# ccchengff/SketchML

Measured on AMD Instinct MI355X. Metric: device-resident grad encode GB/s (fp32 in) + decode L2 err, 1/2/4/8 GPU, higher is better.
Workload: dtype f32; 1 GPU; north star: 2^28-float dense gradient bucket per GPU, 256 requested bins, encode; n_per_gpu=268435456, bins=256, rotating_buffers=2, parallelism=dp1

## Files before the change

include/skml.h:

```cpp
#ifndef SKML_H
#define SKML_H

#include <stddef.h>
#include <stdint.h>

#ifdef __cplusplus
extern "C" {
#endif

#define SKML_OK 0
#define SKML_E_ARG 1
#define SKML_E_NAN 2
#define SKML_E_ORDER 3
#define SKML_E_HIP 4
#define SKML_E_RCCL 5
#define SKML_E_OOM 6
#define SKML_E_STATE 7

#define SKML_DENSE_MAGIC 0x444D4B53u
#define SKML_MAX_BINS 65536

typedef struct skml_ctx skml_ctx;

typedef struct skml_params {
// ... 41 lines not shown
#define SKML_K_DECODE 4
#define SKML_K_DECODE_SUM 5
#define SKML_K_SPARSE 6
#define SKML_K_COUNT 7
#define SKML_TIMING_ALL (-1)
int skml_ctx_set_timing(skml_ctx* ctx, int mask);
int skml_ctx_kernel_stats(skml_ctx* ctx, int kid, int64_t* launches, double* total_ms);
int skml_ctx_reset_stats(skml_ctx* ctx);
int skml_debug_leaf_stage(skml_ctx* ctx, const float* x_dev, int64_t n, int stage, int iters,
                          double* avg_ms);
int skml_debug_sparse_scratch_fail(int on);

int skml_debug_sparse_merge_path(void);

#define SKML_FORM_LEAF_SPLIT 0
#define SKML_FORM_DECODE_SUM 1
#define SKML_FORM_PART_BALLOT 2
#define SKML_FORM_RS_ROUNDS 3
#define SKML_FORM_DEC_ROWS_SERIAL 4
#define SKML_FORM_AGG_TILES 5
#define SKML_FORM_AGG_ONE_LANE 6
#define SKML_FORM_RUN_BOUNDS 7
#define SKML_FORM_DEC_LOOKBACK 8
#define SKML_FORM_COUNT 9
int skml_debug_form(int id, int value);
#define SKML_BUILD_AB 1
int skml_build_flags(void);


size_t skml_dense_payload_bytes(int64_t n, int32_t bin_num);

int skml_dense_encode_f32(skml_ctx* ctx, const float* x_dev, int64_t n, const skml_params* params,
                          void* payload_dev, size_t payload_cap);

int skml_dense_encode_f64(skml_ctx* ctx, const double* x_dev, int64_t n, const skml_params* params,
                          void* payload_dev, size_t payload_cap);

int skml_dense_encode_bf16(skml_ctx* ctx, const uint16_t* x_dev, int64_t n, const skml_params* params,
                           void* payload_dev, size_t payload_cap);
int skml_dense_encode_f16(skml_ctx* ctx, const uint16_t* x_dev, int64_t n, const skml_params* params,
                          void* payload_dev, size_t payload_cap);

int skml_dense_encode_uniform_f32(skml_ctx* ctx, const float* x_dev, int64_t n,
                                  const skml_params* params, void* payload_dev, size_t payload_cap);
int skml_dense_encode_uniform_f64(skml_ctx* ctx, const double* x_dev, int64_t n,
                                  const skml_params* params, void* payload_dev, size_t payload_cap);

// ... 186 lines not shown
```

sketchml_amd/_lib.py:

```python
from __future__ import annotations

import contextlib
import ctypes as C
import os

import torch

_HERE = os.path.dirname(os.path.abspath(__file__))
LIB_PATH = os.environ.get("SKML_LIB", os.path.join(_HERE, "lib", "libskml.so"))

SKML_OK = 0
SKML_E_ARG = 1
SKML_E_NAN = 2
SKML_E_ORDER = 3
SKML_E_HIP = 4
SKML_E_RCCL = 5
SKML_E_OOM = 6
SKML_E_STATE = 7
UNIQUE_ID_BYTES = 128
SKML_MAX_BINS = 65536
SKML_FIXED_MAGIC = 0x584D4B53
SKML_QUANTILE = 0
SKML_UNIFORM = 1

# ... 142 lines not shown
    "skml_comm_init_rank": (C.c_int, [vp, u8p, i32, i32, C.POINTER(vp)]),
    "skml_comm_destroy": (C.c_int, [vp]),
    "skml_allgather": (C.c_int, [vp, vp, vp, C.c_size_t, vp]),
}

EXPORTED = tuple(_SIGS)


def _load():
    if not os.path.exists(LIB_PATH):
        raise ImportError(f"sketchml_amd: HIP library not built ({LIB_PATH}); run "
                          f"`python -c 'import __graft_entry__ as g; g.build()'`")
    lib = C.CDLL(LIB_PATH)
    for name, (res, args) in _SIGS.items():
        fn = getattr(lib, name)
        fn.restype = res
        fn.argtypes = args
    return lib


lib = _load()

FORMS = {"leaf_split": 0, "decode_sum": 1, "part_ballot": 2, "rs_rounds": 3, "dec_rows_serial": 4,
         "agg_tiles": 5, "agg_one_lane": 6, "run_bounds": 7, "dec_lookback": 8}


AB_BUILD = bool(lib.skml_build_flags() & 1)


class FormNotBuilt(RuntimeError):
    """A kernel form only the A/B build carries (skml_debug_form returned -2)."""


@contextlib.contextmanager
def forced_forms(**values):
    prev = {}
    try:
        for k, v in values.items():
            r = lib.skml_debug_form(FORMS[k], int(v))
            if r == -2:
                raise FormNotBuilt(f"form {k}={v} is built only with -DSKML_AB (SKML_LIB=sketchml_amd/lib_ab/libskml.so)")
            if r < 0:
                raise ValueError(f"unknown form {k}")
            prev[k] = r
        yield
    finally:
        for k, v in prev.items():
# ... 6 lines not shown
```

sketchml_amd/csrc/skml_api.cpp:

```cpp
#include <hip/hip_runtime.h>
#include <rccl/rccl.h>

#include <atomic>
#include <cmath>
#include <condition_variable>
#include <cstdarg>
#include <cstdio>
#include <cstdlib>
#include <cstring>
#include <functional>
#include <mutex>
#include <string>
#include <thread>
#include <vector>

#include "skml_internal.h"
#include "skml_sparse.h"

using namespace skml;

namespace {

thread_local std::string g_err;

// ... 10 lines not shown
#define HIP_TRY(expr)                                                                       \
    do {                                                                                    \
        hipError_t e_ = (expr);                                                             \
        if (e_ != hipSuccess)                                                               \
            return fail(SKML_E_HIP, "%s failed: %s (%s:%d)", #expr, hipGetErrorString(e_), \
                        __FILE__, __LINE__);                                                \
    } while (0)

}

struct skml_ctx {
    int device = 0;
    hipStream_t stream = nullptr;
    bool own_stream = false;
    uint64_t* jump_tab = nullptr;
    void* ws = nullptr;
    size_t ws_cap = 0;
    void* ws64 = nullptr;
    size_t ws64_cap = 0;
    int64_t* ranks = nullptr;
    size_t ranks_cap = 0;
    int64_t ranks_n = -1;
    int ranks_bins = -1;
    skml_ctx* side = nullptr;
    hipEvent_t ev_join = nullptr, ev_leaf = nullptr;
    hipEvent_t ev_fork2 = nullptr, ev_join2 = nullptr;
    hipEvent_t after_leaf = nullptr;
    hipEvent_t ev_switch = nullptr;
    void* sk = nullptr;
    size_t sk_cap = 0;
    FxPartial* fx_part = nullptr;
    void* stage = nullptr;
    size_t stage_cap = 0;
    void* scratch[kScratchSlots] = {};
    size_t scratch_cap[kScratchSlots] = {};
    void* pinned = nullptr;
    size_t pinned_cap = 0;
    int64_t* hword = nullptr;
    void* hx = nullptr;
    size_t hx_cap = 0;
    void* hp = nullptr;
    size_t hp_cap = 0;
    void* hk = nullptr;
    size_t hk_cap = 0;
    void* hpin[2] = {nullptr, nullptr};
    size_t hpin_cap = 0;
// ... 25 lines not shown
    }
    ~KernelTimer() {
        if (!on) return;
        (void)hipEventRecord(c->ev[kid][c->ev_used[kid] + 1], c->stream);
        c->ev_used[kid] += 2;
    }
};
KernelTimer* make_timer(skml_ctx* c, int kid) { return new KernelTimer(c, kid); }
void end_timer(KernelTimer* t) { delete t; }

static std::atomic<int> g_form[SKML_FORM_COUNT];
int form(int id) { return id >= 0 && id < SKML_FORM_COUNT ? g_form[id].load(std::memory_order_relaxed) : 0; }
}

static bool ab_only_form(int id, int v) {
    switch (id) {
        case SKML_FORM_LEAF_SPLIT: return v == 1 || v >= 3;
        case SKML_FORM_DECODE_SUM: return v == 2;
        case SKML_FORM_RS_ROUNDS: return v == 2;
        case SKML_FORM_DEC_ROWS_SERIAL: return v == 2;
        case SKML_FORM_AGG_TILES: return v >= 2;
        case SKML_FORM_RUN_BOUNDS: return v != 0;
        case SKML_FORM_DEC_LOOKBACK: return v != 0;
        default: return false;
    }
}

extern "C" int skml_debug_form(int id, int value) {
    if (id < 0 || id >= SKML_FORM_COUNT) return -1;
#ifndef SKML_AB
    if (ab_only_form(id, value)) return -2;
#else
    (void)ab_only_form;
#endif
    return g_form[id].exchange(value);
}

extern "C" int skml_build_flags(void) {
#ifdef SKML_AB
    return SKML_BUILD_AB;
#else
    return 0;
#endif
}

namespace {

struct Workspace {
    unsigned* done;
    LeafPartial* part;
    float* nodes6;
    float* roots;
    float* upA;
    float* upB;
    double* raw;
    QuantLut* lut;
    UniPartial* uni;
    int* qflags;
    uint8_t* ubits;
    LeafPartial* part_red;
};

size_t ws_layout(int64_t chunks, Workspace* w, char* base) {
    const int64_t nwg = (chunks + kLeafChunks - 1) / kLeafChunks;
    const int64_t full = chunks / kLeafChunks;
    const int64_t up = (full >> kMergeGroupLog) + 2 * kMaxLevels + 8;
    size_t off = 0;
    auto take = [&](size_t bytes) {
        size_t o = off;
        off = align_up(off + bytes, 256);
        return base ? (void*)(base + o) : nullptr;
    };
    Workspace t;
    t.done = (unsigned*)take(256);
    t.part = (LeafPartial*)take(sizeof(LeafPartial) * (size_t)(nwg + 1));
    t.nodes6 = (float*)take(sizeof(float) * kK * (size_t)(full + 1));
    t.roots = (float*)take(sizeof(float) * kK * kMaxLevels);
    t.upA = (float*)take(sizeof(float) * kK * (size_t)up);
    t.upB = (float*)take(sizeof(float) * kK * (size_t)up);
    t.raw = (double*)take(sizeof(double) * SKML_MAX_BINS);
    t.lut = (QuantLut*)take(sizeof(QuantLut));
    t.uni = (UniPartial*)take(sizeof(UniPartial) * kUniMaxParts);
    t.qflags = (int*)take(sizeof(int) * 4);
    t.ubits = (uint8_t*)take((size_t)upper_node_count(full * kLeafChunks) + 64);
    t.part_red = (LeafPartial*)take(sizeof(LeafPartial) * (size_t)(full + 8));
    if (w) *w = t;
    return off;
}

int ensure_ws(skml_ctx* ctx, int64_t chunks, Workspace* w) {
    const size_t need = ws_layout(chunks, nullptr, nullptr);
    if (need > ctx->ws_cap) {
        if (ctx->ws) HIP_TRY(hipFree(ctx->ws));
        ctx->ws = nullptr;
        size_t cap = need + need / 4;
        HIP_TRY(hipMalloc(&ctx->ws, cap));
        HIP_TRY(hipMemsetAsync(ctx->ws, 0, 256, ctx->stream));
        ctx->ws_cap = cap;
    }
    ws_layout(chunks, w, (char*)ctx->ws);
    return SKML_OK;
}

struct Workspace64 {
    LeafPartial64* part;
    double* nodes6;
    double* roots;
    double* upA;
    double* upB;
    double* raw;
    uint8_t* ubits;
};

size_t ws64_layout(int64_t chunks, Workspace64* w, char* base) {
    const int64_t tiles = (chunks + kLeafChunks - 1) / kLeafChunks;
    const int64_t up = (tiles >> 3) + 8;
    size_t off = 0;
    auto take = [&](size_t bytes) {
        size_t o = off;
        off = align_up(off + bytes, 256);
// ... 55 lines not shown
        uint64_t a = 1, c = 0;
        for (int b = 0; b < 256; b++) {
            tab[(lvl * 256 + b) * 2] = a;
            tab[(lvl * 256 + b) * 2 + 1] = c;
            c = (base_a * c + base_c) & kLcgMask;
            a = (base_a * a) & kLcgMask;
        }
        uint64_t na = 1, nc = 0;
        for (int i = 0; i < 256; i++) {
            nc = (base_a * nc + base_c) & kLcgMask;
            na = (base_a * na) & kLcgMask;
        }
        base_a = na;
        base_c = nc;
    }
}

struct Tree {
    int level;
    int m;
    int cur_level;
    int64_t src;
    int64_t chunk_base;
};

bool valid_payload_ptr(const void* p) { return p && (((uintptr_t)p) % 256 == 0); }

void destroy_host_path(skml_ctx* c);

}

extern "C" {

void skml_params_default(skml_params* p) {
    p->bin_num = 256;
    p->group_num = 8;
    p->row_num = 2;
    p->dedup = 1;
    p->col_ratio = 0.3;
    p->seed = 0;
    p->hash_seed = 0;
    p->quant_type = SKML_QUANTILE;
    p->parallelism = 1;
}

const char* skml_last_error(void) { return g_err.c_str(); }
// ... 25 lines not shown
    void* pin = e == hipSuccess ? skml::ctx_pinned(c, tab_bytes) : nullptr;
    if (e == hipSuccess && !pin) e = hipErrorOutOfMemory;
    if (e == hipSuccess) {
        std::memcpy(pin, tab.data(), tab_bytes);
        e = hipMemcpyAsync(c->jump_tab, pin, tab_bytes, hipMemcpyHostToDevice, c->stream);
    }
    if (e == hipSuccess) e = hipStreamSynchronize(c->stream);
    if (e != hipSuccess) {
        skml_ctx_destroy(c);
        return fail(SKML_E_HIP, "jump table: %s", hipGetErrorString(e));
    }
    *out = c;
    return SKML_OK;
}

int skml_ctx_destroy(skml_ctx* c) {
    if (!c) return SKML_OK;
    (void)hipSetDevice(c->device);
    if (c->stream) (void)hipStreamSynchronize(c->stream);
    if (c->jump_tab) (void)hipFree(c->jump_tab);
    if (c->ws) (void)hipFree(c->ws);
    if (c->ws64) (void)hipFree(c->ws64);
    if (c->ranks) (void)hipFree(c->ranks);
    if (c->stage) (void)hipFree(c->stage);
    if (c->side) skml_ctx_destroy(c->side);
    if (c->ev_join) (void)hipEventDestroy(c->ev_join);
    if (c->ev_leaf) (void)hipEventDestroy(c->ev_leaf);
    if (c->ev_fork2) (void)hipEventDestroy(c->ev_fork2);
    if (c->ev_join2) (void)hipEventDestroy(c->ev_join2);
    if (c->ev_switch) (void)hipEventDestroy(c->ev_switch);
    if (c->sk) (void)hipFree(c->sk);
    if (c->fx_part) (void)hipFree(c->fx_part);
    for (int k = 0; k < SKML_K_COUNT; k++)
        for (hipEvent_t e : c->ev[k]) (void)hipEventDestroy(e);
    for (int i = 0; i < kScratchSlots; i++)
        if (c->scratch[i]) (void)hipFree(c->scratch[i]);
    if (c->pinned) (void)hipHostFree(c->pinned);
    if (c->hword) (void)hipHostFree(c->hword);
    destroy_host_path(c);
    if (c->own_stream) (void)hipStreamDestroy(c->stream);
    delete c;
    return SKML_OK;
}

int skml_ctx_sync(skml_ctx* c) {
    if (!c) return fail(SKML_E_ARG, "ctx is NULL");
// ... 79 lines not shown
size_t skml_dense_payload_bytes(int64_t n, int32_t bin_num) {
    if (n < 0 || bin_num < 2 || bin_num > SKML_MAX_BINS) return 0;
    const size_t rounded = align_up((size_t)n, 1024);
    return dense_codes_offset(bin_num) + align_up(rounded * (size_t)code_bits_for(bin_num) / 8, 256);
}

static int check_dense_args(skml_ctx* c, const void* x, int64_t n, int bins, const void* payload,
                            size_t cap) {
    if (!c) return fail(SKML_E_ARG, "ctx is NULL");
    if (n < 0 || n > 0x7FFFFFFFLL) return fail(SKML_E_ARG, "n=%lld outside Java int range", (long long)n);
    if (bins < 2 || bins > SKML_MAX_BINS)
        return fail(SKML_E_ARG, "Invalid partition number: %d", bins);
    if (n > 0 && (!x || ((uintptr_t)x) % 16 != 0))
        return fail(SKML_E_ARG, "input must be a 16-byte aligned device pointer");
    if (!valid_payload_ptr(payload)) return fail(SKML_E_ARG, "payload must be 256-byte aligned");
    if (cap < skml_dense_payload_bytes(n, bins))
        return fail(SKML_E_ARG, "payload capacity %zu < %zu", cap, skml_dense_payload_bytes(n, bins));
    return SKML_OK;
}

}

namespace {
std::vector<MergePass> plan_merge_passes(int64_t chunks) {
    std::vector<Tree> trees;
    for (int l = kMaxLevels - 1; l > kLeafTopLevel; l--) {
        if (!((chunks >> l) & 1)) continue;
        Tree t;
        t.level = l;
        t.m = l - kLeafTopLevel;
        t.cur_level = kLeafTopLevel;
        t.chunk_base = (chunks >> (l + 1)) << (l + 1);
        t.src = t.chunk_base >> kLeafTopLevel;
        trees.push_back(t);
    }
    std::vector<MergePass> passes;
    while (true) {
        MergePass pass;
        std::memset(&pass, 0, sizeof(pass));
        int64_t dst_off = 0;
        int wg = 0;
        for (auto& t : trees) {
            if (t.m == 0) continue;
            const int g = t.m < kMergeGroupLog ? t.m : kMergeGroupLog;
            MergeJob& j = pass.job[pass.njobs];
            j.src_node = t.src;
            j.dst_node = dst_off;
            j.chunk_base = t.chunk_base;
            j.level_in = t.cur_level;
            j.group_log = g;
            j.groups = 1 << (t.m - g);
            j.root_level = (t.m - g == 0) ? t.level : -1;
            pass.wg_prefix[pass.njobs] = wg;
            wg += j.groups;
            pass.njobs++;
            t.src = dst_off;
            dst_off += j.groups;
            t.m -= g;
            t.cur_level += g;
        }
        if (pass.njobs == 0) break;
        pass.wg_prefix[pass.njobs] = wg;
        passes.push_back(pass);
    }
    return passes;
}
constexpr int kFuseMaxWg = 4;
bool fuse_next_pass(const std::vector<MergePass>& passes, size_t i) {
    return i + 2 == passes.size() && passes[i + 1].wg_prefix[passes[i + 1].njobs] <= kFuseMaxWg;
}
}

namespace {
int run_sketch_f32(skml_ctx* c, const void* x, int64_t n, uint64_t s0, const Workspace& w, const skml_params* p,
                   void* payload, bool summary, bool* fused_out, int xtype = kXF32) {
    const int64_t chunks = n / kChunk;
    const int64_t nwg = (chunks + kLeafChunks - 1) / kLeafChunks;
    bool fused = false;
    if (chunks > 0) {
        {
            KernelTimer kt(c, SKML_K_LEAF);
            HIP_TRY(launch_leaf(c->stream, x, chunks, s0, c->jump_tab, w.part, w.nodes6, w.roots, w.ubits, xtype));
        }
        if (c->after_leaf) {
            HIP_TRY(hipEventRecord(c->after_leaf, c->stream));
            c->after_leaf = nullptr;
        }
        std::vector<MergePass> passes = plan_merge_passes(chunks);
        if (summary && !passes.empty()) passes.back().fuse_summary = 1;
        const int64_t nred = passes.empty() ? 0 : passes[0].wg_prefix[passes[0].njobs];
        const int64_t part_from = passes.empty() ? 0 : (chunks >> 7) << 1;
        const float* src = w.nodes6;
        float* dst = w.upA;
        for (size_t i = 0; i < passes.size(); i++) {
            const bool fuse_next = fuse_next_pass(passes, i);
            float* next_dst = (dst == w.upA) ? w.upB : w.upA;
            KernelTimer kt(c, SKML_K_MERGE);
            HIP_TRY(launch_merge_pass(c->stream, passes[i], fuse_next ? &passes[i + 1] : nullptr, src, dst, next_dst,
                                      w.roots, s0, c->jump_tab, w.done, x, n, w.part, nwg, c->ranks, p->bin_num,
                                      p->dedup ? 1 : 0, payload, w.raw, w.lut, w.ubits,
                                      summary ? w.part_red : nullptr, summary ? nred : 0, summary ? part_from : 0,
                                      xtype));
            src = dst;
            dst = next_dst;
            if (fuse_next) break;
        }
        fused = summary && !passes.empty();
    }
    *fused_out = fused;
    return SKML_OK;
}
// ... 1452 lines not shown
```

sketchml_amd/csrc/skml_internal.h:

```cpp
#pragma once
#include <hip/hip_runtime.h>
#include <stddef.h>
#include <stdint.h>

#include "../../include/skml.h"

namespace skml {

int form(int id);

enum XType : int { kXF32 = 0, kXBF16 = 1, kXF16 = 2 };
struct bf16_t { uint16_t bits; };
struct f16_t { uint16_t bits; };

constexpr uint64_t kLcgMult = 0x5DEECE66DULL;
constexpr uint64_t kLcgAdd = 0xBULL;
constexpr uint64_t kLcgMask = (1ULL << 48) - 1;

constexpr int kK = 128;
constexpr int kChunk = 2 * kK;
constexpr int kLeafWaves = 8;
constexpr int kChunksPerWave = 8;
constexpr int kLeafChunks = kLeafWaves * kChunksPerWave;
constexpr int kLeafTopLevel = 6;
// ... 41 lines not shown
};

struct SketchRecord64 {
    int64_t n;
    LeafPartial64 mm;
    double tail[kChunk];
    double level[kMaxLevels][kK];
};
hipError_t launch_leaf2_f64(hipStream_t st, const double* x, int64_t chunks, uint64_t s0, const uint64_t* jump_tab,
                            LeafPartial64* part, double* nodes6, double* roots, uint8_t* ubits);
hipError_t launch_sketch_record64(hipStream_t st, const double* x, int64_t n, const LeafPartial64* part,
                                  int64_t nparts, const double* roots, SketchRecord64* rec);
hipError_t launch_sketch_merge64(hipStream_t st, const SketchRecord64* recs, int nrec, uint64_t s0, uint64_t bit0,
                                 const uint64_t* jump_tab, double* roots, double* tail, LeafPartial64* part);

struct MergeJob {
    int64_t src_node;
    int64_t dst_node;
    int64_t chunk_base;
    int32_t level_in;
    int32_t group_log;
    int32_t groups;
    int32_t root_level;
};
constexpr int kMaxJobs = 24;
struct MergePass {
    MergeJob job[kMaxJobs];
    int32_t njobs;
    int32_t fuse_summary;
    int32_t wg_prefix[kMaxJobs + 1];
};

__host__ __device__ inline size_t align_up(size_t x, size_t a) { return (x + a - 1) / a * a; }
__host__ __device__ inline int code_bits_for(int bins) {
    int b = 1;
    while ((1LL << b) < bins) b <<= 1;
    return b;
}
__host__ __device__ inline size_t dense_codes_offset(int req_bins) {
    return align_up(kHeaderBytes + 8 * (size_t)(req_bins - 1), 256);
}

__host__ __device__ inline int64_t upper_level_offset(int64_t C, int L) {
    int64_t o = 0;
    for (int l = kLeafTopLevel + 1; l < L; l++) o += C >> l;
    return o;
}
__host__ __device__ inline int64_t upper_node_count(int64_t C) { return upper_level_offset(C, kMaxLevels); }

hipError_t launch_leaf(hipStream_t st, const void* x, int64_t chunks, uint64_t s0,
                       const uint64_t* jump_tab, LeafPartial* part, float* nodes6, float* roots, uint8_t* ubits,
                       int xtype = kXF32);
hipError_t launch_leaf_stage(hipStream_t st, int stage, const float* x, int64_t chunks, uint64_t s0,
                             const uint64_t* jump_tab, LeafPartial* part, float* scratch, float* roots);
hipError_t launch_merge_pass64(hipStream_t st, const MergePass& pass, const MergePass* next, const double* src,
                               double* dst, double* next_dst, double* roots, uint64_t s0, const uint64_t* jump_tab,
                               unsigned* done, const uint8_t* ubits, int64_t uchunks);
hipError_t launch_sketch_record(hipStream_t st, const float* x, int64_t n, const LeafPartial* part, int64_t nparts,
                                const float* roots, SketchRecord* rec);
hipError_t launch_sketch_merge(hipStream_t st, const SketchRecord* recs, int nrec, uint64_t s0, uint64_t bit0,
                               const uint64_t* jump_tab, int64_t n_total, int64_t n_local, const int64_t* ranks,
                               int req_bins, int dedup, void* payload, double* scratch_raw, QuantLut* lut,
                               float* scratch_roots, float* scratch_tail, LeafPartial* scratch_part);
hipError_t launch_merge_pass(hipStream_t st, const MergePass& pass, const MergePass* next, const float* src,
                             float* dst, float* next_dst, float* roots, uint64_t s0, const uint64_t* jump_tab,
                             unsigned* done, const void* x, int64_t n, const LeafPartial* part, int64_t nparts,
                             const int64_t* ranks, int req_bins, int dedup, void* payload,
                             double* scratch_raw, QuantLut* lut, const uint8_t* ubits, LeafPartial* part_red,
                             int64_t nred, int64_t part_from, int xtype = kXF32);
hipError_t launch_summary(hipStream_t st, const void* x, int64_t n, const LeafPartial* part,
                          int64_t nparts, const float* roots, const int64_t* ranks, int req_bins,
                          int dedup, void* payload, double* scratch_raw, QuantLut* lut, int xtype = kXF32);
hipError_t launch_set_ranks(hipStream_t st, int64_t n, int bins, int64_t* ranks);
hipError_t launch_set_splits(hipStream_t st, void* payload, int64_t n, const double* splits_dev,
                             int nsplits, double mn, double mx, int req_bins, QuantLut* lut);
hipError_t launch_quantize(hipStream_t st, const void* x, int64_t n, void* payload, const QuantLut* lut,
                           int req_bins, int xtype = kXF32);
hipError_t launch_decode(hipStream_t st, const void* payload, void* out, int64_t n, int otype = kXF32);
hipError_t launch_decode_sum(hipStream_t st, const void* payloads, int P, size_t stride, void* out,
                             int64_t n, double scale, int common_bits,
                             int max_bins, int otype = kXF32);
hipError_t launch_bins(hipStream_t st, const void* payload, int32_t* bins, int64_t n);
hipError_t launch_ref_body(hipStream_t st, const void* payload, uint8_t* out, int64_t n, int width);
hipError_t launch_times_by(hipStream_t st, void* payload, double x);
constexpr int kFxHeaderBytes = 256;
constexpr int kFxMinBits = 2, kFxMaxBits = 29;
constexpr int kFxMaxParts = 1024;
struct FxPartial {
    double sum;
    uint32_t flags;
    uint32_t pad;
};
// ... 27 lines not shown
```

sketchml_amd/csrc/skml_sketch.hip:

```cpp
#include <cstdlib>
#include <cstring>
#include <type_traits>

#include "skml_device.hpp"

namespace skml {

__device__ unsigned long long g_prof[32];
#ifdef SKML_PROF_LEAF
__device__ unsigned long long g_leafprof[4 * 65536];
#endif
#ifdef SKML_PROF_SUMMARY
#define SKML_PROF(k)                                      \
    do {                                                  \
        if (threadIdx.x == 0) g_prof[(k)] = wall_clock64(); \
    } while (0)
#else
#define SKML_PROF(k) \
    do {             \
    } while (0)
#endif

constexpr int kWaveFb = 1536;
template <typename S>
// ... 1185 lines not shown
        const double fmin = (double)__uint_as_float(key2f(S.min_key));
        const double fmax = (double)__uint_as_float(key2f(S.max_key));
        if (fmin <= vmin) vmin = fmin;
        if (fmax > vmax) vmax = fmax;
    }
    if (S.flags & 1u) {
        payload_zero_tail(a.payload, 0, req_bins);
        if (t == 0) {
            hdr->magic = SKML_DENSE_MAGIC;
            hdr->status = SKML_E_NAN;
            hdr->n = a.sharded ? a.n_local : n;
            hdr->bin_num = req_bins;
            hdr->zero_idx = 0;
            hdr->code_bits = code_bits_for(req_bins);
            hdr->req_bins = req_bins;
            hdr->min = vmin;
            hdr->max = vmax;
            hdr->codes_offset = (int64_t)dense_codes_offset(req_bins);
            hdr->reserved = 0;
        }
        return;
    }

    {
        const int nfull = nruns - 1;
        const float* tail_run = S.smp + S.run_off[nfull];
        for (int i = t; i < ns; i += T) {
            const int r = i < nfull * kK ? i / kK : nfull;
            const float v = S.smp[i];
            int rank = i - S.run_off[r];
            for (int q0 = 0; q0 < nfull; q0 += 2) {
                const int q1 = q0 + 1 < nfull ? q0 + 1 : q0;
                const uint32_t use_a = (uint32_t)(q0 != r), use_b = (uint32_t)(q1 != r) & (uint32_t)(q1 != q0);
                if (!(use_a | use_b)) continue;
                rank += rank_in_run_pair(S.smp + q0 * kK, S.smp + q1 * kK, v, (uint32_t)(q0 < r),
                                         (uint32_t)(q1 < r), use_a, use_b);
            }
            if (r < nfull) rank += run_count_lt(tail_run, tail, v);
            S.sorted[rank] = v;
            S.w[rank] = S.run_lvl[r] < 0 ? 1 : ((int64_t)2 << S.run_lvl[r]);
        }
    }
    __syncthreads();
    SKML_PROF(5);

    {
        const int per = (ns + T - 1) / T;
        const int b0 = min(ns, t * per), b1 = min(ns, b0 + per);
        int64_t loc = 0;
        for (int i = b0; i < b1; i++) loc += S.w[i];
        const int64_t base = block_scan_excl(loc, S.wsum, &S.total);
        int64_t acc = base;
        for (int i = b0; i < b1; i++) {
            const int64_t wv = S.w[i];
            S.w[i] = acc;
            acc += wv;
        }
        if (t == 0) S.w[ns] = S.total;
    }
    __syncthreads();
    SKML_PROF(6);

    const int nsplit_req = req_bins - 1;
    const bool lds_raw = nsplit_req <= kSumMaxRaw;
    double* raw = lds_raw ? S.raw : a.g_raw;
    for (int i = t; i < nsplit_req; i += T) {
        double sp;
        if (ns == 0) {
            sp = __longlong_as_double(0x7FF8000000000000LL);
        } else {
            const int64_t rank = has_rank ? pre_rank : a.ranks[i];
            int lo = 0, hi = ns;
            while (lo + 1 < hi) {
                const int mid = (lo + hi) >> 1;
                if (S.w[mid] <= rank) lo = mid;
                else hi = mid;
            }
            sp = (double)S.sorted[lo];
        }
        raw[i] = sp;
    }
    if (!lds_raw) __threadfence();
    __syncthreads();
    SKML_PROF(7);

    int bin_num;
    {
        const int per = (nsplit_req + T - 1) / T;
        const int b0 = min(nsplit_req, t * per), b1 = min(nsplit_req, b0 + per);
        int64_t loc = 0;
        for (int i = b0; i < b1; i++) loc += (!a.dedup || i == 0 || raw[i] != raw[i - 1]) ? 1 : 0;
        const int64_t base = block_scan_excl(loc, S.wsum, &S.total);
        int64_t o = base;
        int zmin = 0x7FFFFFFF;
        for (int i = b0; i < b1; i++) {
            if (!a.dedup || i == 0 || raw[i] != raw[i - 1]) {
                const double sp = raw[i];
                splits[o] = sp;
                if (o < kMaxSamples) S.smp[o] = (float)sp;
                if (!(sp < 0.0)) zmin = min(zmin, (int)o);
                o++;
// ... 51 lines not shown
}

hipError_t launch_summary(hipStream_t st, const void* x, int64_t n, const LeafPartial* part,
                          int64_t nparts, const float* roots, const int64_t* ranks, int req_bins,
                          int dedup, void* payload, double* scratch_raw, QuantLut* lut, int xtype) {
    SummaryArgs a{x, n, part, nparts, roots, ranks, reinterpret_cast<uint8_t*>(payload), scratch_raw,
                  lut, req_bins, dedup};
    a.xtype = xtype;
    hipLaunchKernelGGL(k_summary, dim3(1), dim3(512), 0, st, a);
    return hipGetLastError();
}

template <typename S = float>
struct MergeExport {
    int lane, wave, g;
    S* out;
    template <int R, typename T>
    __device__ __forceinline__ void at(int level, int node, const T (&w)[R]) const {
        if (level == g && wave == 0 && node == 0) store_node<R>(w, lane, out);
    }
};

template <typename E = float>
__device__ __forceinline__ void merge_group_wg(const MergePass& pass, int wg, const E* __restrict__ src,
                                               E* __restrict__ dst, E* __restrict__ roots, uint64_t s0,
                                               const uint64_t* __restrict__ tab, TileSharedT<E>& sh,
                                               const uint8_t* __restrict__ ubits, int64_t uchunks,
                                               const LeafPartial* __restrict__ part_in = nullptr,
                                               LeafPartial* __restrict__ part_red = nullptr, int prof = -1) {
#ifdef SKML_PROF_SUMMARY
#define SKML_PROF_AT(k)                                                  \
    do {                                                                 \
        if (prof >= 0 && threadIdx.x == 0) g_prof[prof + (k)] = wall_clock64(); \
    } while (0)
#else
#define SKML_PROF_AT(k) \
    do {                \
    } while (0)
#endif
    SKML_PROF_AT(0);
    using T = typename std::conditional<std::is_same<E, double>::value, double, uint32_t>::type;
    const int tid = threadIdx.x, wave = tid >> 6, lane = tid & 63;
    int j = 0;
    while (j + 1 < pass.njobs && wg >= pass.wg_prefix[j + 1]) j++;
    const MergeJob job = pass.job[j];
    const int grp = wg - pass.wg_prefix[j];
    const int g = job.group_log, L = job.level_in;
    const int nodes = 1 << g;
    const int64_t node0 = job.src_node + ((int64_t)grp << g);
    const int64_t chunk0 = job.chunk_base + ((int64_t)grp << (g + L));
    E* out = job.root_level >= 0 ? roots + (size_t)job.root_level * kK : dst + (size_t)(job.dst_node + grp) * kK;
    if constexpr (!std::is_same<E, double>::value) {
        if (g == 2 && !(part_red && L == kLeafTopLevel)) {
            if (wave != 0) return;
            uint32_t bsel = 0;
            if (lane < 3) {
                const int lo = lane < 2 ? 1 : 2, last_node = lane < 2 ? 2 * lane + 1 : 3;
                const int lvl = L + lo;
                const int64_t i = ((chunk0 + ((int64_t)(last_node + 1) << L)) >> lvl) - 1;
                const int64_t cnt = upper_node_count(uchunks);
                int64_t idx = upper_level_offset(uchunks, lvl) + i;
                idx = idx < cnt ? idx : cnt - 1;
                bsel = ubits[idx < 0 ? 0 : idx];
            }
            const float4* p = reinterpret_cast<const float4*>(src + (size_t)(node0 + (lane >> 4)) * kK) + (lane & 15) * 2;
            T w1[8], w2[4], w3[2];
            uint32_t fl = 0;
#pragma unroll
            for (int q = 0; q < 2; q++) {
// ... 17 lines not shown
            SKML_PROF_AT(3);
            return;
        }
    }
    if (tid == 0) sh.flags = 0u;
    uint32_t bsel = 0;
    {
        int lo = -1, last_node = 0;
        if (lane < 4) lo = 1, last_node = wave * 8 + 2 * lane + 1;
        else if (lane < 6) lo = 2, last_node = wave * 8 + 4 * (lane - 4) + 3;
        else if (lane == 6) lo = 3, last_node = wave * 8 + 7;
        else if (wave == 0 && lane >= 8 && lane < 12) lo = 4, last_node = 16 * (lane - 8) + 15;
        else if (wave == 0 && lane >= 12 && lane < 14) lo = 5, last_node = 32 * (lane - 12) + 31;
        else if (wave == 0 && lane == 14) lo = 6, last_node = 63;
        if (lo > 0) {
            const int lvl = L + lo;
            const int64_t i = ((chunk0 + ((int64_t)(last_node + 1) << L)) >> lvl) - 1;
            const int64_t cnt = upper_node_count(uchunks);
            int64_t idx = upper_level_offset(uchunks, lvl) + i;
            idx = idx < cnt ? idx : cnt - 1;
            bsel = ubits[idx < 0 ? 0 : idx];
        }
    }
    (void)tab;
    (void)s0;
    const bool reduce_parts = part_red && L == kLeafTopLevel && wave == 0;
    LeafPartial tp{0xFFFFFFFFu, 0u, 0u, 0u};
    if (reduce_parts && lane < nodes) tp = part_in[node0 + lane];
    __syncthreads();

    const int nd = wave * 8 + (lane >> 3);
    const bool valid = nd < nodes;
    T w1[16];
    uint32_t fl = 0;
    if constexpr (std::is_same<E, double>::value) {
        const double2* p = reinterpret_cast<const double2*>(src + (size_t)(node0 + (valid ? nd : 0)) * kK) + (lane & 7) * 8;
#pragma unroll
        for (int q = 0; q < 8; q++) {
            const double2 f = p[q];
            const double e2[2] = {f.x, f.y};
#pragma unroll
            for (int e = 0; e < 2; e++) {
                const uint64_t b = (uint64_t)__double_as_longlong(e2[e]);
                fl |= (b == 0x8000000000000000ull) ? 2u : 0u;
                fl |= (b == 0ull) ? 4u : 0u;
                w1[q * 2 + e] = e2[e];
            }
        }
// ... 29 lines not shown
    {
        const uint64_t m = __ballot(bsel != 0);
        ibits = (uint32_t)m & 0x7Fu;
        if (wave == 0 && lane == 0) sh.wgbits = (uint32_t)(m >> 8) & 0x7Fu;
    }
#ifdef SKML_PROF_SUMMARY
    if (prof == 16 && threadIdx.x == 0) g_prof[22] = wall_clock64();
#endif
    if (fl) atomicOr(&sh.flags, fl);
    const bool wexact = (__ballot((fl & 2u) != 0) != 0) && (__ballot((fl & 4u) != 0) != 0);
    const MergeExport<E> exp{lane, wave, g, out};
    T w4[2];
    inwave_levels(w1, w4, lane, ibits, wexact, sh.fb[wave], exp, prof == 16);
    store_node<2>(w4, lane, sh.wn[wave]);
    __syncthreads();
    SKML_PROF_AT(2);
    if (g >= 4) {
        crosswave_levels<T>(sh, tid, sh.wgbits, (sh.flags & 6u) == 6u);
        if (tid < kK) out[tid] = g == 4 ? sh.l4[0][tid] : (g == 5 ? sh.l5[0][tid] : sh.l6[tid]);
    }
    SKML_PROF_AT(3);
}

__global__ __launch_bounds__(512) void k_merge(MergePass pass, MergePass next, const float* __restrict__ src,
                                               float* __restrict__ dst, float* __restrict__ next_dst,
                                               float* __restrict__ roots, uint64_t s0,
                                               const uint64_t* __restrict__ tab, unsigned* __restrict__ done,
                                               SummaryArgs sa, const uint8_t* __restrict__ ubits, int64_t uchunks) {
    __shared__ MergeShared U;
    const int tid = threadIdx.x;
    if (pass.fuse_summary && gridDim.x == 1) SKML_PROF(0);
    merge_group_wg(pass, (int)blockIdx.x, src, dst, roots, s0, tab, U.t, ubits, uchunks, sa.part,
                   const_cast<LeafPartial*>(sa.part_red), blockIdx.x == 0 ? 12 : -1);
    const bool has_next = next.njobs > 0;
    if (!pass.fuse_summary && !has_next) return;

    asm volatile("s_waitcnt vmcnt(0)" ::: "memory");
    __syncthreads();
    if (tid == 0) {
        __builtin_amdgcn_fence(__ATOMIC_RELEASE, "agent");
        asm volatile("s_waitcnt vmcnt(0)" ::: "memory");
        const unsigned old = atomicAdd(done, 1u);
        const int last = old == (unsigned)(pass.wg_prefix[pass.njobs] - 1);
        if (last) {
#ifdef SKML_PROF_SUMMARY
            g_prof[20] = wall_clock64();
#endif
            *done = 0u;
            __builtin_amdgcn_fence(__ATOMIC_ACQUIRE, "agent");
            asm volatile("s_waitcnt vmcnt(0)" ::: "memory");
#ifdef SKML_PROF_SUMMARY
            g_prof[21] = wall_clock64();
#endif
        }
        U.t.is_last = last;
    }
    __syncthreads();
    if (!U.t.is_last) return;
    __syncthreads();
    LeafPartial pre{0xFFFFFFFFu, 0u, 0u, 0u};
    const int64_t npre = sa.nred + (sa.nparts - sa.part_from);
    const bool prefetch = pass.fuse_summary || next.fuse_summary ? npre <= (int64_t)blockDim.x : false;
    if (prefetch && tid < npre) pre = tid < sa.nred ? sa.part_red[tid] : sa.part[sa.part_from + (tid - sa.nred)];
    const int nsplit = sa.req_bins - 1;
    const bool rank_ahead = (pass.fuse_summary || next.fuse_summary) && nsplit <= (int)blockDim.x;
    int64_t pre_rank = 0;
    if (rank_ahead && tid < nsplit) pre_rank = sa.ranks[tid];
    if (has_next) {
        SKML_PROF(0);
        const int nnext = next.wg_prefix[next.njobs];
        for (int w = 0; w < nnext; w++) {
            if (w) __syncthreads();
            merge_group_wg(next, w, dst, next_dst, roots, s0, tab, U.t, ubits, uchunks, nullptr, nullptr,
                           w == 0 ? 16 : -1);
        }
        asm volatile("s_waitcnt vmcnt(0)" ::: "memory");
        __builtin_amdgcn_fence(__ATOMIC_SEQ_CST, "workgroup");
        __syncthreads();
        if (!next.fuse_summary) return;
    }
    SKML_PROF(1);
    summary_block(sa, U.s, prefetch, pre, rank_ahead, pre_rank);
#ifdef SKML_PROF_WARM
    __syncthreads();
    if (threadIdx.x == 0) g_prof[26] = wall_clock64();
    summary_block(sa, U.s);
    __syncthreads();
    if (threadIdx.x == 0) g_prof[27] = wall_clock64();
#endif
}

hipError_t launch_merge_pass(hipStream_t st, const MergePass& pass, const MergePass* next, const float* src,
                             float* dst, float* next_dst, float* roots, uint64_t s0, const uint64_t* jump_tab,
                             unsigned* done, const void* x, int64_t n, const LeafPartial* part, int64_t nparts,
                             const int64_t* ranks, int req_bins, int dedup, void* payload,
                             double* scratch_raw, QuantLut* lut, const uint8_t* ubits, LeafPartial* part_red,
                             int64_t nred, int64_t part_from, int xtype) {
    const int nwg = pass.wg_prefix[pass.njobs];
    if (nwg <= 0) return hipSuccess;
    SummaryArgs a{x, n, part, nparts, roots, ranks, reinterpret_cast<uint8_t*>(payload), scratch_raw,
                  lut, req_bins, dedup};
    a.xtype = xtype;
    a.part_red = part_red;
    a.nred = nred;
    a.part_from = part_from;
    MergePass none;
    if (!next) {
        std::memset(&none, 0, sizeof(none));
        next = &none;
    }
    const int64_t uchunks = (n / kChunk / kLeafWaveChunks) * kLeafWaveChunks;
    hipLaunchKernelGGL(k_merge, dim3(nwg), dim3(512), 0, st, pass, *next, src, dst, next_dst, roots, s0, jump_tab,
                       done, a, ubits, uchunks);
    return hipGetLastError();
}

__global__ __launch_bounds__(512) void k_merge64(MergePass pass, MergePass next, const double* __restrict__ src,
                                                 double* __restrict__ dst, double* __restrict__ next_dst,
                                                 double* __restrict__ roots, uint64_t s0,
                                                 const uint64_t* __restrict__ tab, unsigned* __restrict__ done,
                                                 const uint8_t* __restrict__ ubits, int64_t uchunks) {
    __shared__ TileSharedT<double> T64;
    const int tid = threadIdx.x;
    merge_group_wg<double>(pass, (int)blockIdx.x, src, dst, roots, s0, tab, T64, ubits, uchunks);
    if (next.njobs == 0) return;
    asm volatile("s_waitcnt vmcnt(0)" ::: "memory");
    __syncthreads();
    if (tid == 0) {
        __builtin_amdgcn_fence(__ATOMIC_RELEASE, "agent");
        asm volatile("s_waitcnt vmcnt(0)" ::: "memory");
        const unsigned old = atomicAdd(done, 1u);
        const int last = old == (unsigned)(pass.wg_prefix[pass.njobs] - 1);
        if (last) {
            *done = 0u;
            __builtin_amdgcn_fence(__ATOMIC_ACQUIRE, "agent");
            asm volatile("s_waitcnt vmcnt(0)" ::: "memory");
        }
        T64.is_last = last;
    }
// ... 273 lines not shown
```

Before: 1911 GB/s.

## Add chained single-launch merge form and single-run summary fast path

Adds an A/B-only merge-chain kernel that runs all merge passes in one launch. It uses per-group arrival counters so the last workgroup of each group continues to the next level, which removes a separate launch per pass. It also adds a group-cap form knob and enlarges the done-counter region. In the default build, the summary gets a fast path that, when there is exactly one run and no tail, indexes splits directly instead of building weights and binary searching. The merge job lookup is also simplified for job 0.

```diff
diff --git a/include/skml.h b/include/skml.h
--- a/include/skml.h
+++ b/include/skml.h
@@ -87,7 +87,9 @@
 #define SKML_FORM_AGG_ONE_LANE 6
 #define SKML_FORM_RUN_BOUNDS 7
 #define SKML_FORM_DEC_LOOKBACK 8
-#define SKML_FORM_COUNT 9
+#define SKML_FORM_MERGE_CHAIN 9
+#define SKML_FORM_MERGE_GROUP_CAP 10
+#define SKML_FORM_COUNT 11
 int skml_debug_form(int id, int value);
 #define SKML_BUILD_AB 1
 int skml_build_flags(void);
diff --git a/sketchml_amd/_lib.py b/sketchml_amd/_lib.py
--- a/sketchml_amd/_lib.py
+++ b/sketchml_amd/_lib.py
@@ -188,7 +188,8 @@
 lib = _load()
 
 FORMS = {"leaf_split": 0, "decode_sum": 1, "part_ballot": 2, "rs_rounds": 3, "dec_rows_serial": 4,
-         "agg_tiles": 5, "agg_one_lane": 6, "run_bounds": 7, "dec_lookback": 8}
+         "agg_tiles": 5, "agg_one_lane": 6, "run_bounds": 7, "dec_lookback": 8, "merge_chain": 9,
+         "merge_group_cap": 10}
 
 
 AB_BUILD = bool(lib.skml_build_flags() & 1)
diff --git a/sketchml_amd/csrc/skml_api.cpp b/sketchml_amd/csrc/skml_api.cpp
--- a/sketchml_amd/csrc/skml_api.cpp
+++ b/sketchml_amd/csrc/skml_api.cpp
@@ -56,6 +56,13 @@
     size_t ranks_cap = 0;
     int64_t ranks_n = -1;
     int ranks_bins = -1;
+#ifdef SKML_AB
+    skml::MergePass* plan_dev = nullptr;
+    int64_t plan_chunks = -1;
+    int plan_gmax = -1;
+    skml::MergePass plan_pass0;
+    skml::MergeChain plan_chain;
+#endif
     skml_ctx* side = nullptr;
     hipEvent_t ev_join = nullptr, ev_leaf = nullptr;
     hipEvent_t ev_fork2 = nullptr, ev_join2 = nullptr;
@@ -127,6 +134,7 @@
         case SKML_FORM_AGG_TILES: return v >= 2;
         case SKML_FORM_RUN_BOUNDS: return v != 0;
         case SKML_FORM_DEC_LOOKBACK: return v != 0;
+        case SKML_FORM_MERGE_CHAIN: return v != 0;
         default: return false;
     }
 }
@@ -166,10 +174,15 @@
     LeafPartial* part_red;
 };
 
+int merge_group_max() {
+    const int cap = form(SKML_FORM_MERGE_GROUP_CAP);
+    return cap == 2 || cap == 3 ? cap : kMergeGroupLog;
+}
+
 size_t ws_layout(int64_t chunks, Workspace* w, char* base) {
     const int64_t nwg = (chunks + kLeafChunks - 1) / kLeafChunks;
     const int64_t full = chunks / kLeafChunks;
-    const int64_t up = (full >> kMergeGroupLog) + 2 * kMaxLevels + 8;
+    const int64_t up = (full >> merge_group_max()) + 2 * kMaxLevels + 8;
     size_t off = 0;
     auto take = [&](size_t bytes) {
         size_t o = off;
@@ -177,7 +190,7 @@
         return base ? (void*)(base + o) : nullptr;
     };
     Workspace t;
-    t.done = (unsigned*)take(256);
+    t.done = (unsigned*)take(sizeof(unsigned) * kMaxArrivals);
     t.part = (LeafPartial*)take(sizeof(LeafPartial) * (size_t)(nwg + 1));
     t.nodes6 = (float*)take(sizeof(float) * kK * (size_t)(full + 1));
     t.roots = (float*)take(sizeof(float) * kK * kMaxLevels);
@@ -200,7 +213,7 @@
         ctx->ws = nullptr;
         size_t cap = need + need / 4;
         HIP_TRY(hipMalloc(&ctx->ws, cap));
-        HIP_TRY(hipMemsetAsync(ctx->ws, 0, 256, ctx->stream));
+        HIP_TRY(hipMemsetAsync(ctx->ws, 0, sizeof(unsigned) * kMaxArrivals, ctx->stream));
         ctx->ws_cap = cap;
     }
     ws_layout(chunks, w, (char*)ctx->ws);
@@ -302,6 +315,7 @@
     int cur_level;
     int64_t src;
     int64_t chunk_base;
+    int job;
 };
 
 bool valid_payload_ptr(const void* p) { return p && (((uintptr_t)p) % 256 == 0); }
@@ -373,6 +387,9 @@
     if (c->ws) (void)hipFree(c->ws);
     if (c->ws64) (void)hipFree(c->ws64);
     if (c->ranks) (void)hipFree(c->ranks);
+#ifdef SKML_AB
+    if (c->plan_dev) (void)hipFree(c->plan_dev);
+#endif
     if (c->stage) (void)hipFree(c->stage);
     if (c->side) skml_ctx_destroy(c->side);
     if (c->ev_join) (void)hipEventDestroy(c->ev_join);
@@ -498,7 +515,7 @@
 }
 
 namespace {
-std::vector<MergePass> plan_merge_passes(int64_t chunks) {
+std::vector<MergePass> plan_merge_passes(int64_t chunks, int gmax = kMergeGroupLog) {
     std::vector<Tree> trees;
     for (int l = kMaxLevels - 1; l > kLeafTopLevel; l--) {
         if (!((chunks >> l) & 1)) continue;
@@ -508,6 +525,7 @@
         t.cur_level = kLeafTopLevel;
         t.chunk_base = (chunks >> (l + 1)) << (l + 1);
         t.src = t.chunk_base >> kLeafTopLevel;
+        t.job = -1;
         trees.push_back(t);
     }
     std::vector<MergePass> passes;
@@ -518,7 +536,7 @@
         int wg = 0;
         for (auto& t : trees) {
             if (t.m == 0) continue;
-            const int g = t.m < kMergeGroupLog ? t.m : kMergeGroupLog;
+            const int g = t.m < gmax ? t.m : gmax;
             MergeJob& j = pass.job[pass.njobs];
             j.src_node = t.src;
             j.dst_node = dst_off;
@@ -527,6 +545,16 @@
             j.group_log = g;
             j.groups = 1 << (t.m - g);
             j.root_level = (t.m - g == 0) ? t.level : -1;
+#ifdef SKML_AB
+            j.next_job = j.next_first = j.next_glog = -1;
+            if (t.job >= 0) {
+                MergeJob& prev = passes.back().job[t.job];
+                prev.next_job = pass.njobs;
+                prev.next_first = wg;
+                prev.next_glog = g;
+            }
+#endif
+            t.job = pass.njobs;
             pass.wg_prefix[pass.njobs] = wg;
             wg += j.groups;
             pass.njobs++;
@@ -545,6 +573,43 @@
 bool fuse_next_pass(const std::vector<MergePass>& passes, size_t i) {
     return i + 2 == passes.size() && passes[i + 1].wg_prefix[passes[i + 1].njobs] <= kFuseMaxWg;
 }
+
+#ifdef SKML_AB
+int ensure_plan(skml_ctx* ctx, int64_t chunks) {
+    const int gmax = merge_group_max();
+    if (ctx->plan_chunks == chunks && ctx->plan_gmax == gmax) return SKML_OK;
+    const std::vector<MergePass> passes = plan_merge_passes(chunks, gmax);
+    MergeChain ch;
+    std::memset(&ch, 0, sizeof(ch));
+    std::memset(&ctx->plan_pass0, 0, sizeof(MergePass));
+    ch.npasses = (int)passes.size();
+    if (ch.npasses > kMaxPasses) return fail(SKML_E_ARG, "merge plan: %d passes", ch.npasses);
+    int nctr = 0, pass0_trees = 0;
+    for (int i = 0; i < ch.npasses; i++) {
+        const MergePass& ps = passes[i];
+        if (i > 0) {
+            ch.ctr_base[i] = nctr;
+            nctr += ps.wg_prefix[ps.njobs];
+        }
+        for (int j = 0; j < ps.njobs; j++) ch.nroots += ps.job[j].root_level >= 0 ? 1 : 0;
+    }
+    ch.final_ctr = nctr++;
+    if (nctr > kMaxArrivals) return fail(SKML_E_ARG, "merge plan: %d arrival counters (the group cap form is for small n)", nctr);
+    if (ch.npasses > 0) {
+        pass0_trees = passes[0].njobs;
+        ctx->plan_pass0 = passes[0];
+    }
+    ch.single_tree = pass0_trees == 1;
+    if (ch.npasses > 1) {
+        if (!ctx->plan_dev) HIP_TRY(hipMalloc(&ctx->plan_dev, sizeof(MergePass) * kMaxPasses));
+        for (int i = 1; i < ch.npasses; i++) HIP_TRY(launch_store_pass(ctx->stream, passes[i], ctx->plan_dev + i));
+    }
+    ctx->plan_chain = ch;
+    ctx->plan_chunks = chunks;
+    ctx->plan_gmax = gmax;
+    return SKML_OK;
+}
+#endif
 }
 
 namespace {
@@ -562,7 +627,25 @@
             HIP_TRY(hipEventRecord(c->after_leaf, c->stream));
             c->after_leaf = nullptr;
         }
-        std::vector<MergePass> passes = plan_merge_passes(chunks);
+#ifdef SKML_AB
+        if (form(SKML_FORM_MERGE_CHAIN) == 1) {
+            if (int st = ensure_plan(c, chunks)) return st;
+            const MergeChain& ch = c->plan_chain;
+            if (ch.npasses > 0) {
+                MergePass pass0 = c->plan_pass0;
+                pass0.fuse_summary = summary ? 1 : 0;
+                const int64_t nred0 = pass0.wg_prefix[pass0.njobs];
+                KernelTimer kt(c, SKML_K_MERGE);
+                HIP_TRY(launch_merge_chain(c->stream, pass0, ch, c->plan_dev, w.nodes6, w.upA, w.upB, w.roots, w.done, x,
+                                           n, w.part, nwg, c->ranks, p->bin_num, p->dedup ? 1 : 0, payload, w.raw, w.lut,
+                                           w.ubits, summary ? w.part_red : nullptr, summary ? nred0 : 0,
+                                           summary ? (chunks >> 7) << 1 : 0, xtype));
+            }
+            *fused_out = summary && ch.npasses > 0;
+            return SKML_OK;
+        }
+#endif
+        std::vector<MergePass> passes = plan_merge_passes(chunks, merge_group_max());
         if (summary && !passes.empty()) passes.back().fuse_summary = 1;
         const int64_t nred = passes.empty() ? 0 : passes[0].wg_prefix[passes[0].njobs];
         const int64_t part_from = passes.empty() ? 0 : (chunks >> 7) << 1;
diff --git a/sketchml_amd/csrc/skml_internal.h b/sketchml_amd/csrc/skml_internal.h
--- a/sketchml_amd/csrc/skml_internal.h
+++ b/sketchml_amd/csrc/skml_internal.h
@@ -87,6 +87,12 @@
     int32_t group_log;
     int32_t groups;
     int32_t root_level;
+#ifdef SKML_AB
+    int32_t next_job;
+    int32_t next_first;
+    int32_t next_glog;
+    int32_t pad;
+#endif
 };
 constexpr int kMaxJobs = 24;
 struct MergePass {
@@ -94,6 +100,19 @@
     int32_t njobs;
     int32_t fuse_summary;
     int32_t wg_prefix[kMaxJobs + 1];
+};
+constexpr int kMaxPasses = 9;
+#ifdef SKML_AB
+constexpr int kMaxArrivals = 4096;
+#else
+constexpr int kMaxArrivals = 64;
+#endif
+struct MergeChain {
+    int32_t npasses;
+    int32_t nroots;
+    int32_t single_tree;
+    int32_t final_ctr;
+    int32_t ctr_base[kMaxPasses];
 };
 
 __host__ __device__ inline size_t align_up(size_t x, size_t a) { return (x + a - 1) / a * a; }
@@ -133,6 +152,14 @@
                              const int64_t* ranks, int req_bins, int dedup, void* payload,
                              double* scratch_raw, QuantLut* lut, const uint8_t* ubits, LeafPartial* part_red,
                              int64_t nred, int64_t part_from, int xtype = kXF32);
+#ifdef SKML_AB
+hipError_t launch_merge_chain(hipStream_t st, const MergePass& pass0, const MergeChain& chain, const MergePass* later,
+                              const float* nodes6, float* upA, float* upB, float* roots, unsigned* ctr, const void* x,
+                              int64_t n, const LeafPartial* part, int64_t nparts, const int64_t* ranks, int req_bins,
+                              int dedup, void* payload, double* scratch_raw, QuantLut* lut, const uint8_t* ubits,
+                              LeafPartial* part_red, int64_t nred, int64_t part_from, int xtype = kXF32);
+hipError_t launch_store_pass(hipStream_t st, const MergePass& pass, MergePass* dst);
+#endif
 hipError_t launch_summary(hipStream_t st, const void* x, int64_t n, const LeafPartial* part,
                           int64_t nparts, const float* roots, const int64_t* ranks, int req_bins,
                           int dedup, void* payload, double* scratch_raw, QuantLut* lut, int xtype = kXF32);
diff --git a/sketchml_amd/csrc/skml_sketch.hip b/sketchml_amd/csrc/skml_sketch.hip
--- a/sketchml_amd/csrc/skml_sketch.hip
+++ b/sketchml_amd/csrc/skml_sketch.hip
@@ -1231,7 +1231,9 @@
         return;
     }
 
-    {
+    const bool one_run = tail == 0 && nruns == 2;
+    const int one_shift = S.run_lvl[0] + 1;
+    if (!one_run) {
         const int nfull = nruns - 1;
         const float* tail_run = S.smp + S.run_off[nfull];
         for (int i = t; i < ns; i += T) {
@@ -1250,10 +1252,10 @@
             S.w[rank] = S.run_lvl[r] < 0 ? 1 : ((int64_t)2 << S.run_lvl[r]);
         }
     }
-    __syncthreads();
+    if (!one_run) __syncthreads();
     SKML_PROF(5);
 
-    {
+    if (!one_run) {
         const int per = (ns + T - 1) / T;
         const int b0 = min(ns, t * per), b1 = min(ns, b0 + per);
         int64_t loc = 0;
@@ -1267,7 +1269,7 @@
         }
         if (t == 0) S.w[ns] = S.total;
     }
-    __syncthreads();
+    if (!one_run) __syncthreads();
     SKML_PROF(6);
 
     const int nsplit_req = req_bins - 1;
@@ -1279,13 +1281,18 @@
             sp = __longlong_as_double(0x7FF8000000000000LL);
         } else {
             const int64_t rank = has_rank ? pre_rank : a.ranks[i];
-            int lo = 0, hi = ns;
-            while (lo + 1 < hi) {
-                const int mid = (lo + hi) >> 1;
-                if (S.w[mid] <= rank) lo = mid;
-                else hi = mid;
-            }
-            sp = (double)S.sorted[lo];
+            if (one_run) {
+                const int64_t idx = rank >> one_shift;
+                sp = (double)S.smp[idx < ns - 1 ? (int)idx : ns - 1];
+            } else {
+                int lo = 0, hi = ns;
+                while (lo + 1 < hi) {
+                    const int mid = (lo + hi) >> 1;
+                    if (S.w[mid] <= rank) lo = mid;
+                    else hi = mid;
+                }
+                sp = (double)S.sorted[lo];
+            }
         }
         raw[i] = sp;
     }
@@ -1383,12 +1390,11 @@
 };
 
 template <typename E = float>
-__device__ __forceinline__ void merge_group_wg(const MergePass& pass, int wg, const E* __restrict__ src,
-                                               E* __restrict__ dst, E* __restrict__ roots, uint64_t s0,
-                                               const uint64_t* __restrict__ tab, TileSharedT<E>& sh,
-                                               const uint8_t* __restrict__ ubits, int64_t uchunks,
-                                               const LeafPartial* __restrict__ part_in = nullptr,
-                                               LeafPartial* __restrict__ part_red = nullptr, int prof = -1) {
+__device__ __forceinline__ void merge_job_wg(const MergeJob& job, int grp, int wg, const E* __restrict__ src,
+                                             E* __restrict__ dst, E* __restrict__ roots, TileSharedT<E>& sh,
+                                             const uint8_t* __restrict__ ubits, int64_t uchunks,
+                                             const LeafPartial* __restrict__ part_in = nullptr,
+                                             LeafPartial* __restrict__ part_red = nullptr, int prof = -1) {
 #ifdef SKML_PROF_SUMMARY
 #define SKML_PROF_AT(k)                                                  \
     do {                                                                 \
@@ -1402,10 +1408,6 @@
     SKML_PROF_AT(0);
     using T = typename std::conditional<std::is_same<E, double>::value, double, uint32_t>::type;
     const int tid = threadIdx.x, wave = tid >> 6, lane = tid & 63;
-    int j = 0;
-    while (j + 1 < pass.njobs && wg >= pass.wg_prefix[j + 1]) j++;
-    const MergeJob job = pass.job[j];
-    const int grp = wg - pass.wg_prefix[j];
     const int g = job.group_log, L = job.level_in;
     const int nodes = 1 << g;
     const int64_t node0 = job.src_node + ((int64_t)grp << g);
@@ -1469,8 +1471,6 @@
             bsel = ubits[idx < 0 ? 0 : idx];
         }
     }
-    (void)tab;
-    (void)s0;
     const bool reduce_parts = part_red && L == kLeafTopLevel && wave == 0;
     LeafPartial tp{0xFFFFFFFFu, 0u, 0u, 0u};
     if (reduce_parts && lane < nodes) tp = part_in[node0 + lane];
@@ -1546,17 +1546,48 @@
     SKML_PROF_AT(3);
 }
 
+__device__ __forceinline__ int pass_job_of(const MergePass& pass, int wg) {
+    int j = 0;
+    while (j + 1 < pass.njobs && wg >= pass.wg_prefix[j + 1]) j++;
+    return j;
+}
+template <typename E = float>
+__device__ __forceinline__ void merge_group_wg(const MergePass& pass, int wg, const E* __restrict__ src,
+                                               E* __restrict__ dst, E* __restrict__ roots, uint64_t s0,
+                                               const uint64_t* __restrict__ tab, TileSharedT<E>& sh,
+                                               const uint8_t* __restrict__ ubits, int64_t uchunks,
+                                               const LeafPartial* __restrict__ part_in = nullptr,
+                                               LeafPartial* __restrict__ part_red = nullptr, int prof = -1) {
+    (void)tab;
+    (void)s0;
+    const int njobs = pass.njobs, first1 = pass.wg_prefix[1];
+    MergeJob job = pass.job[0];
+    int base = 0;
+    if (njobs > 1 && wg >= first1) {
+        const int j = pass_job_of(pass, wg);
+        job = pass.job[j];
+        base = pass.wg_prefix[j];
+    }
+    merge_job_wg<E>(job, wg - base, wg, src, dst, roots, sh, ubits, uchunks, part_in, part_red, prof);
+}
+
 __global__ __launch_bounds__(512) void k_merge(MergePass pass, MergePass next, const float* __restrict__ src,
                                                float* __restrict__ dst, float* __restrict__ next_dst,
                                                float* __restrict__ roots, uint64_t s0,
                                                const uint64_t* __restrict__ tab, unsigned* __restrict__ done,
                                                SummaryArgs sa, const uint8_t* __restrict__ ubits, int64_t uchunks) {
     __shared__ MergeShared U;
+    __shared__ int s_last;
     const int tid = threadIdx.x;
     if (pass.fuse_summary && gridDim.x == 1) SKML_PROF(0);
+    const bool has_next = next.njobs > 0;
+    const int nnext = next.wg_prefix[next.njobs];
+    const MergeJob next_job0 = next.job[0];
+    const int64_t npre = sa.nred + (sa.nparts - sa.part_from);
+    const int nsplit = sa.req_bins - 1;
+    const bool ahead = pass.fuse_summary || next.fuse_summary;
     merge_group_wg(pass, (int)blockIdx.x, src, dst, roots, s0, tab, U.t, ubits, uchunks, sa.part,
                    const_cast<LeafPartial*>(sa.part_red), blockIdx.x == 0 ? 12 : -1);
-    const bool has_next = next.njobs > 0;
     if (!pass.fuse_summary && !has_next) return;
 
     asm volatile("s_waitcnt vmcnt(0)" ::: "memory");
@@ -1577,26 +1608,22 @@
             g_prof[21] = wall_clock64();
 #endif
         }
-        U.t.is_last = last;
-    }
-    __syncthreads();
-    if (!U.t.is_last) return;
-    __syncthreads();
+        s_last = last;
+    }
+    __syncthreads();
+    if (!s_last) return;
     LeafPartial pre{0xFFFFFFFFu, 0u, 0u, 0u};
-    const int64_t npre = sa.nred + (sa.nparts - sa.part_from);
-    const bool prefetch = pass.fuse_summary || next.fuse_summary ? npre <= (int64_t)blockDim.x : false;
+    const bool prefetch = ahead ? npre <= (int64_t)blockDim.x : false;
     if (prefetch && tid < npre) pre = tid < sa.nred ? sa.part_red[tid] : sa.part[sa.part_from + (tid - sa.nred)];
-    const int nsplit = sa.req_bins - 1;
-    const bool rank_ahead = (pass.fuse_summary || next.fuse_summary) && nsplit <= (int)blockDim.x;
+    const bool rank_ahead = ahead && nsplit <= (int)blockDim.x;
     int64_t pre_rank = 0;
     if (rank_ahead && tid < nsplit) pre_rank = sa.ranks[tid];
     if (has_next) {
         SKML_PROF(0);
-        const int nnext = next.wg_prefix[next.njobs];
-        for (int w = 0; w < nnext; w++) {
-            if (w) __syncthreads();
-            merge_group_wg(next, w, dst, next_dst, roots, s0, tab, U.t, ubits, uchunks, nullptr, nullptr,
-                           w == 0 ? 16 : -1);
+        merge_job_wg(next_job0, 0, 0, dst, next_dst, roots, U.t, ubits, uchunks, nullptr, nullptr, 16);
+        for (int w = 1; w < nnext; w++) {
+            __syncthreads();
+            merge_group_wg(next, w, dst, next_dst, roots, s0, tab, U.t, ubits, uchunks);
         }
         asm volatile("s_waitcnt vmcnt(0)" ::: "memory");
         __builtin_amdgcn_fence(__ATOMIC_SEQ_CST, "workgroup");
@@ -1639,6 +1666,123 @@
     return hipGetLastError();
 }
 
+#ifdef SKML_AB
+__global__ __launch_bounds__(512) void k_merge_chain(MergePass pass0, MergeChain chain,
+                                                     const MergePass* __restrict__ later,
+                                                     const float* __restrict__ nodes6, float* __restrict__ upA,
+                                                     float* __restrict__ upB, float* __restrict__ roots,
+                                                     unsigned* __restrict__ ctr, SummaryArgs sa,
+                                                     const uint8_t* __restrict__ ubits, int64_t uchunks) {
+    __shared__ MergeShared U;
+    __shared__ int s_last;
+    const int tid = threadIdx.x;
+    int wg = (int)blockIdx.x;
+    const int j0 = pass_job_of(pass0, wg);
+    MergeJob job = pass0.job[j0];
+    int grp = wg - pass0.wg_prefix[j0];
+    const bool summary = pass0.fuse_summary != 0;
+    MergeJob nj = job;
+    if (job.next_job >= 0) nj = later[1].job[job.next_job];
+    if (summary && gridDim.x == 1) SKML_PROF(0);
+    merge_job_wg(job, grp, wg, nodes6, upA, roots, U.t, ubits, uchunks, sa.part, const_cast<LeafPartial*>(sa.part_red),
+                 blockIdx.x == 0 ? 12 : -1);
+    LeafPartial pre{0xFFFFFFFFu, 0u, 0u, 0u};
+    bool prefetch = false, rank_ahead = false;
+    int64_t pre_rank = 0;
+    const float* src = upA;
+    float* dst = upB;
+    for (int p = 0;; p++) {
+        const bool root = job.next_job < 0;
+        if (root && !summary) return;
+        if (root && chain.nroots == 1) {
+            asm volatile("s_waitcnt vmcnt(0)" ::: "memory");
+            __builtin_amdgcn_fence(__ATOMIC_SEQ_CST, "workgroup");
+            __syncthreads();
+            break;
+        }
+        const int cw = root ? 0 : job.next_first + (grp >> job.next_glog);
+        unsigned* c = ctr + (root ? chain.final_ctr : chain.ctr_base[p + 1] + cw);
+        const unsigned need = root ? (unsigned)chain.nroots : 1u << job.next_glog;
+        const bool stamp = root || p + 2 == chain.npasses;
+        (void)stamp;
+        asm volatile("s_waitcnt vmcnt(0)" ::: "memory");
+        __syncthreads();
+        if (tid == 0) {
+            __builtin_amdgcn_fence(__ATOMIC_RELEASE, "agent");
+            asm volatile("s_waitcnt vmcnt(0)" ::: "memory");
+            const unsigned old = atomicAdd(c, 1u);
+            const int last = old == need - 1u;
+            if (last) {
+#ifdef SKML_PROF_SUMMARY
+                if (stamp) g_prof[20] = wall_clock64();
+#endif
+                *c = 0u;
+                __builtin_amdgcn_fence(__ATOMIC_ACQUIRE, "agent");
+                asm volatile("s_waitcnt vmcnt(0)" ::: "memory");
+#ifdef SKML_PROF_SUMMARY
+                if (stamp) g_prof[21] = wall_clock64();
+                if (p == 0 && !stamp) g_prof[11] = wall_clock64();
+#endif
+            }
+            s_last = last;
+        }
+        __syncthreads();
+        if (!s_last) return;
+        if (root) break;
+        grp >>= job.next_glog;
+        job = nj;
+        wg = cw;
+        if (job.next_job >= 0) nj = later[p + 2].job[job.next_job];
+        const bool top = p + 2 == chain.npasses;
+        if (top && summary && chain.single_tree) {
+            const int64_t npre = sa.nred + (sa.nparts - sa.part_from);
+            prefetch = npre <= (int64_t)blockDim.x;
+            if (prefetch && tid < npre) pre = tid < sa.nred ? sa.part_red[tid] : sa.part[sa.part_from + (tid - sa.nred)];
+            const int nsplit = sa.req_bins - 1;
+            rank_ahead = nsplit <= (int)blockDim.x;
+            if (rank_ahead && tid < nsplit) pre_rank = sa.ranks[tid];
+        }
+        if (top) SKML_PROF(0);
+        merge_job_wg(job, grp, wg, src, dst, roots, U.t, ubits, uchunks, nullptr, nullptr, top ? 16 : -1);
+        const float* t = src;
+        src = dst;
+        dst = const_cast<float*>(t);
+    }
+    SKML_PROF(1);
+    summary_block(sa, U.s, prefetch, pre, rank_ahead, pre_rank);
+}
+
+hipError_t launch_merge_chain(hipStream_t st, const MergePass& pass0, const MergeChain& chain, const MergePass* later,
+                              const float* nodes6, float* upA, float* upB, float* roots, unsigned* ctr, const void* x,
+                              int64_t n, const LeafPartial* part, int64_t nparts, const int64_t* ranks, int req_bins,
+                              int dedup, void* payload, double* scratch_raw, QuantLut* lut, const uint8_t* ubits,
+                              LeafPartial* part_red, int64_t nred, int64_t part_from, int xtype) {
+    const int nwg = pass0.wg_prefix[pass0.njobs];
+    if (nwg <= 0) return hipSuccess;
+    SummaryArgs a{x, n, part, nparts, roots, ranks, reinterpret_cast<uint8_t*>(payload), scratch_raw,
+                  lut, req_bins, dedup};
+    a.xtype = xtype;
+    a.part_red = part_red;
+    a.nred = nred;
+    a.part_from = part_from;
+    const int64_t uchunks = (n / kChunk / kLeafWaveChunks) * kLeafWaveChunks;
+    hipLaunchKernelGGL(k_merge_chain, dim3(nwg), dim3(512), 0, st, pass0, chain, later, nodes6, upA, upB, roots, ctr, a,
+                       ubits, uchunks);
+    return hipGetLastError();
+}
+
+__global__ __launch_bounds__(64) void k_store_pass(MergePass pass, MergePass* __restrict__ dst) {
+    static_assert(sizeof(MergePass) % sizeof(uint32_t) == 0, "MergePass is copied by words");
+    const uint32_t* s = reinterpret_cast<const uint32_t*>(&pass);
+    uint32_t* d = reinterpret_cast<uint32_t*>(dst);
+    for (int i = threadIdx.x; i < (int)(sizeof(MergePass) / sizeof(uint32_t)); i += 64) d[i] = s[i];
+}
+hipError_t launch_store_pass(hipStream_t st, const MergePass& pass, MergePass* dst) {
+    hipLaunchKernelGGL(k_store_pass, dim3(1), dim3(64), 0, st, pass, dst);
+    return hipGetLastError();
+}
+#endif
+
 __global__ __launch_bounds__(512) void k_merge64(MergePass pass, MergePass next, const double* __restrict__ src,
                                                  double* __restrict__ dst, double* __restrict__ next_dst,
                                                  double* __restrict__ roots, uint64_t s0,
```

Result: no change. 1923 GB/s (median of 6 runs) (+0.6%).
